# kaigu1997/gaussian_process_liouville_equation

Hardware: AMD Instinct MI355X
Metric: GP fit+predict ms/step (N samples, M grid pts) (lower is better)
Workload: dtype f64

## Files before the change

### gaussian_process_liouville_equation_amd/csrc/gple_capi.h

```cpp
#pragma once
#include <atomic>
#include <condition_variable>
#include <cstring>
#include <functional>
#include <limits>
#include <mutex>
#include <vector>

#include "gple_kernels.h"

using namespace gple;

struct gple_ctx: gple::Ctx
{
	struct PoolEntry
	{
		void* p;
		size_t bytes;
		bool used;
	};
	std::vector<PoolEntry> pool;
	std::mutex pool_mu;
	std::mutex call_mu;
	std::atomic<int> refs{1};
	std::atomic<bool> closed{false};

	double* acquire(size_t bytes, hipError_t* err)
	{
		std::lock_guard<std::mutex> lk(pool_mu);
		*err = hipSuccess;
		if (bytes == 0) bytes = 8;
		PoolEntry* best = nullptr;
		for (PoolEntry& e : pool)
			if (!e.used && e.bytes >= bytes && e.bytes <= 2 * bytes + 4096 && (!best || e.bytes < best->bytes)) best = &e;
		if (best)
		{
			best->used = true;
			return static_cast<double*>(best->p);
		}
		void* p = nullptr;
		*err = hipMalloc(&p, bytes);
		if (*err != hipSuccess) return nullptr;
		pool.push_back({p, bytes, true});
		return static_cast<double*>(p);
	}
	void give_back(void* p)
	{
		if (!p) return;
		std::lock_guard<std::mutex> lk(pool_mu);
		for (PoolEntry& e : pool)
			if (e.p == p) e.used = false;
	}
};

inline void ctx_retain(gple_ctx* c) { c->refs.fetch_add(1); }
inline void ctx_drop(gple_ctx* ctx)
{
	if (ctx->refs.fetch_sub(1) != 1) return;
	(void)hipSetDevice(ctx->device);
	(void)hipStreamSynchronize(ctx->stream);
	for (auto& e : ctx->pool) (void)hipFree(e.p);
	if (ctx->host_scalars) (void)hipHostFree(ctx->host_scalars);
	if (ctx->prune_stats) (void)hipFree(ctx->prune_stats);
	if (ctx->format_table) (void)hipFree(ctx->format_table);
	if (ctx->dag_flags) (void)hipFree(ctx->dag_flags);
	timer_collect(ctx);
	for (hipEvent_t e : ctx->ev_free) (void)hipEventDestroy(e);
	if (ctx->side_stream)
	{
		(void)hipStreamSynchronize(ctx->side_stream);
		(void)hipStreamDestroy(ctx->side_stream);
		for (hipEvent_t ev : ctx->side_forks) (void)hipEventDestroy(ev);
		if (ctx->side_join) (void)hipEventDestroy(ctx->side_join);
	}
	if (ctx->owns_stream) (void)hipStreamDestroy(ctx->stream);
	delete ctx;
}
#define GPLE_OPEN(ctx)                                  \
	do                                                  \
	{                                                   \
		if ((ctx)->closed.load()) return GPLE_ERR_STATE; \
	} while (0)
#define GPLE_CALL(ctx)                                             \
	std::lock_guard<std::mutex> gple_call_lk_((ctx)->call_mu); \
	GPLE_HIP((ctx), hipSetDevice((ctx)->device))

namespace gple
{
	constexpr int SDEV_N = 512;
	constexpr int HS_PRED_ERR = 512, HS_PRED_DERIV = 520, HS_NLML = 540;
	constexpr int SDEV_INFO = 31;
	constexpr int HS_FEW_XS = 600, HS_FEW_LAB = 640, HS_FEW_MEAN = 680, HS_FEW_VAR = 720, HS_FEW_CUT = 740;
	constexpr size_t FEW_HOST_POINTS = 16;

	struct Scratch
	{
		gple_ctx* ctx;
		double* p = nullptr;
		explicit Scratch(gple_ctx* c): ctx(c) {}
		Scratch(const Scratch&) = delete;
		~Scratch() { ctx->give_back(p); }
		hipError_t get(size_t doubles)
		{
			hipError_t e;
			p = ctx->acquire(doubles * sizeof(double), &e);
			return e;
		}
	};

	inline double nan_() { return std::numeric_limits<double>::quiet_NaN(); }

	inline hipError_t copy_in(hipStream_t s, double* dst, const double* src, size_t n, bool dev)
	{
		if (n == 0) return hipSuccess;
		return hipMemcpyAsync(dst, src, n * sizeof(double), dev ? hipMemcpyDeviceToDevice : hipMemcpyHostToDevice, s);
	}
	inline hipError_t copy_out(hipStream_t s, double* dst, const double* src, size_t n, bool dev)
	{
		if (n == 0 || dst == nullptr) return hipSuccess;
		return hipMemcpyAsync(dst, src, n * sizeof(double), dev ? hipMemcpyDeviceToDevice : hipMemcpyDeviceToHost, s);
	}

	struct Staged
	{
		Scratch buf;
		const bool dev;
		double* p = nullptr;
		double* host = nullptr;
		size_t n = 0;
		Staged(gple_ctx* c, bool device): buf(c), dev(device) {}
		hipError_t in(const double* src, size_t count)
		{
			p = const_cast<double*>(src);
			if (dev || !src) return hipSuccess;
			hipError_t e = buf.get(count);
			p = buf.p;
			return e == hipSuccess ? copy_in(buf.ctx->stream, p, src, count, false) : e;
		}
		hipError_t out(double* dst, size_t count)
		{
			p = dst;
			if (dev || !dst) return hipSuccess;
			host = dst, n = count;
			hipError_t e = buf.get(count);
			p = buf.p;
			return e;
		}
		hipError_t inout(double* a, size_t count)
		{
			if (!dev && a) host = a, n = count;
			return in(a, count);
		}
		hipError_t back() { return host ? copy_out(buf.ctx->stream, host, p, n, false) : hipSuccess; }
	};
}

struct FitCommon
{
	std::atomic<int> refs{1};
	gple_ctx* ctx = nullptr;
	int N = 0, Np = 0, n_total = 0;
	unsigned flags = 0;
	bool is_complex = false;
	double* Xt = nullptr;
	double* ys = nullptr;
	double* T = nullptr;
	double* v = nullptr;
	double* w = nullptr;
	double* wx = nullptr;
	double* W = nullptr;
	double* dv = nullptr;
	double sf = 1.0;
	double s0 = 1.0;
	DSpecSet dspec[6];
	double* sdev = nullptr;
	double s_host = 0.0;
	bool sc_ready = false;
	mutable std::atomic<bool> validated{false};
	mutable std::atomic<bool> recovered{false};
	mutable std::atomic<int> stale_uses{0};
	unsigned deriv_mask = 0xFFu;
	SEParamSet ps{};
	double self = 0.0;
	FitCommon() { std::memset(dspec, 0, sizeof(dspec)); }
	std::mutex lazy_mu;
	struct PointRequest
	{
		const double* x;
		double *mean, *var, *cut;
		int status;
		bool done;
	};
	mutable std::mutex point_mu;
	mutable std::condition_variable point_cv;
	mutable std::vector<PointRequest*> point_pending;
	mutable bool point_leader = false;

	~FitCommon()
	{
		if (!ctx) return;
		for (double* p : {Xt, ys, T, v, w, wx, W, dv, sdev}) ctx->give_back(p);
		ctx_drop(ctx);
	}
};
struct gple_real_fit: FitCommon
{
	double theta[4];
	gple_real_fit_scalars sc;
};
struct gple_complex_fit: FitCommon
{
	double theta[8];
	gple_complex_fit_scalars sc;
};

namespace gple
{
	constexpr unsigned PREDICT_NO_SYNC = 0x10000u;
	void predict_scalars_from_host(gple_ctx* ctx, bool has_labels, bool want_deriv, bool cplx, gple_predict_scalars* scalars);
	int predict_common(gple_ctx* ctx, const FitCommon* f, const double* Xs, size_t M, unsigned flags, const double* labels, double* prediction,
		double* variance, double* cutoff_prediction, gple_predict_scalars* scalars);
	inline bool own_outputs_written(int status, const FitCommon* f) { return status == GPLE_OK || (status == GPLE_ERR_TIMEOUT && f->validated.load()); }
	int real_fit_create_masked(gple_ctx* ctx, const double theta[4], const double* X, const double* y, int y_is_complex, size_t N, unsigned flags,
		unsigned deriv_mask, gple_real_fit_scalars* scalars, gple_real_fit** out);
	int complex_fit_create_masked(gple_ctx* ctx, const double theta[8], const double* X, const double* y, size_t N, unsigned flags, unsigned deriv_mask,
		gple_complex_fit_scalars* scalars, gple_complex_fit** out);
	int fit_predict(gple_ctx* ctx, const FitCommon* fit, const double* Xs, size_t M, unsigned flags, const double* labels, double* prediction,
		double* variance, double* cutoff_prediction, gple_predict_scalars* scalars);
	template <typename F>
	int fit_get_scalars(F* fit, decltype(F::sc)* out);
	template <typename F>
	int fit_release(F* fit);
	int note_give_up(gple_ctx* ctx, int attempt);
	int nlml_solve(gple_ctx* ctx, const double x[5], const double* X, const double* y, size_t N, Scratch& Xt, Scratch& yd, Scratch& T, Scratch& bvec,
		Scratch& info, int* n_out, bool dev = false);
	int nlml_gave_up(gple_ctx* ctx, int attempt, bool* again);
	using PointBatchEval = std::function<void(const std::vector<std::vector<double>>&, std::vector<double>&)>;
	int neldermead_speculative(const PointBatchEval& eval, unsigned n, const double* lb, const double* ub, const gple_opt_options* options, double* x,
		double* fmin, int* n_eval);
}
```

### gaussian_process_liouville_equation_amd/csrc/gple_capi.hip

```cpp
#include <algorithm>
#include <cmath>
#include <new>

#include "gple_capi.h"
#include "gple_debug.h"

namespace gple
{
	int record_hip_error(Ctx* ctx, hipError_t e, const char* what, const char* file, int line)
	{
		if (ctx)
		{
			std::lock_guard<std::mutex> lk(ctx->mu);
			ctx->last_error = std::string(hipGetErrorString(e)) + " in " + what + " (" + file + ":" + std::to_string(line) + ")";
		}
		(void)hipGetLastError();
		return e == hipErrorOutOfMemory ? GPLE_ERR_ALLOC : GPLE_ERR_HIP;
	}
	static bool take_event(Ctx* c, hipEvent_t* e)
	{
		if (!c->ev_free.empty())
		{
			*e = c->ev_free.back();
			c->ev_free.pop_back();
// ... 683 lines not shown
		}
		if (contracted_blocks) *contracted_blocks = h[0];
		if (seen_blocks) *seen_blocks = h[1];
		return GPLE_OK;
	}
	int gple_ctx_get_timing(gple_ctx* ctx, gple_timer which, double* last_ms, double* total_ms, long* count)
	{
		if (!ctx || static_cast<int>(which) < 0 || static_cast<int>(which) >= Ctx::NTIMERS) return GPLE_ERR_BAD_ARG;
		GPLE_OPEN(ctx);
		GPLE_CALL(ctx);
		GPLE_HIP(ctx, hipStreamSynchronize(ctx->stream));
		timer_collect(ctx);
		if (last_ms) *last_ms = ctx->t_last[which];
		if (total_ms) *total_ms = ctx->t_total[which];
		if (count) *count = ctx->t_count[which];
		return GPLE_OK;
	}

	int gple_real_gram(gple_ctx* ctx, const double theta[4], const double* left, size_t R, const double* right, size_t C,
		int same_features, unsigned flags, double* K, double* dK)
	{
		if (!ctx || !theta || !K || (R && !left) || (C && !right)) return GPLE_ERR_BAD_ARG;
		GPLE_OPEN(ctx);
		if (R == 0 || C == 0) return GPLE_OK;
		GPLE_CALL(ctx);
		const bool dev = flags & GPLE_IO_DEVICE;
		const SEParam p = make_se(theta[0] * theta[0], theta[3] * theta[3], theta[1], theta[2]);
		Staged l(ctx, dev), r(ctx, dev), k(ctx, dev), dk(ctx, dev);
		GPLE_HIP(ctx, l.in(left, 2 * R));
		GPLE_HIP(ctx, r.in(right, 2 * C));
		GPLE_HIP(ctx, k.out(K, R * C));
		GPLE_HIP(ctx, dk.out(dK, 4 * R * C));
		GPLE_HIP(ctx, launch_gram_rect(ctx->stream, l.p, (int)R, r.p, (int)C, same_features, p, theta[0], theta[3], k.p, dk.p));
		GPLE_HIP(ctx, k.back());
		GPLE_HIP(ctx, dk.back());
		if (!dev) GPLE_HIP(ctx, hipStreamSynchronize(ctx->stream));
		return GPLE_OK;
	}

	int gple_complex_gram(gple_ctx* ctx, const double theta[8], const double* left, size_t R, const double* right, size_t C, int same_features,
		unsigned flags, double* K, double* Kt, double* dK, double* dKt)
	{
		if (!ctx || !theta || !K || (R && !left) || (C && !right)) return GPLE_ERR_BAD_ARG;
		GPLE_OPEN(ctx);
		if (R == 0 || C == 0) return GPLE_OK;
		GPLE_CALL(ctx);
		const bool dev = flags & GPLE_IO_DEVICE;
		const size_t rc = R * C;
		Staged l(ctx, dev), r(ctx, dev), k(ctx, dev), kt(ctx, dev), dk(ctx, dev), dkt(ctx, dev);
		GPLE_HIP(ctx, l.in(left, 2 * R));
		GPLE_HIP(ctx, r.in(right, 2 * C));
		GPLE_HIP(ctx, k.out(K, rc));
		GPLE_HIP(ctx, kt.out(Kt, 2 * rc));
		GPLE_HIP(ctx, dk.out(dK, 8 * rc));
		GPLE_HIP(ctx, dkt.out(dKt, 16 * rc));
		GPLE_HIP(ctx, launch_complex_gram(ctx->stream, theta, l.p, (int)R, r.p, (int)C, same_features, k.p, kt.p, dk.p, dkt.p));
		for (Staged* o : {&k, &kt, &dk, &dkt}) GPLE_HIP(ctx, o->back());
		if (!dev) GPLE_HIP(ctx, hipStreamSynchronize(ctx->stream));
		return GPLE_OK;
	}

	int gple_cutoff_factor(gple_ctx* ctx, const double* prediction, int is_complex, const double* variance, size_t M, unsigned flags,
		double* factor)
	{
		if (!ctx || (M && (!prediction || !variance || !factor))) return GPLE_ERR_BAD_ARG;
		GPLE_OPEN(ctx);
		if (M == 0) return GPLE_OK;
		GPLE_CALL(ctx);
		const bool dev = flags & GPLE_IO_DEVICE;
		Staged p(ctx, dev), v(ctx, dev), f(ctx, dev);
		GPLE_HIP(ctx, p.in(prediction, is_complex ? 2 * M : M));
		GPLE_HIP(ctx, v.in(variance, M));
		GPLE_HIP(ctx, f.out(factor, M));
		GPLE_HIP(ctx, launch_cutoff(ctx->stream, p.p, is_complex, v.p, (int)M, f.p));
		GPLE_HIP(ctx, f.back());
		if (!dev) GPLE_HIP(ctx, hipStreamSynchronize(ctx->stream));
		return GPLE_OK;
	}

}

namespace
{
	static int fit_post(gple_ctx* ctx, gple_real_fit* f)
	{
		hipStream_t st = ctx->stream;
		const unsigned flags = f->flags;
		const double sf = f->theta[0], l0 = f->theta[1], l1 = f->theta[2], sn = f->theta[3];
		const size_t N = f->N;
		Scratch part(ctx);
		const size_t g = (N + 63) / 64;
		const bool avg = (flags & GPLE_CALC_AVERAGE) != 0;
		if (avg)
		{
			GPLE_HIP(ctx, part.get(g * g));
			GPLE_HIP(ctx, launch_quadform_partials(st, f->Xt, f->N, purity_aux(sf, l0, l1), f->v, f->v, -1, part.p));
		}
		GPLE_HIP(ctx, launch_real_fit_sums(st, f->Xt, f->ys, f->v, f->w, f->N, f->sdev + 1, avg ? part.p : nullptr, static_cast<int>(g * g), f->sdev + 6));
		if (flags & GPLE_CALC_DERIVATIVE) GPLE_TRY(real_fit_derivatives(ctx, f, sf, l0, l1, sn, flags));
		return GPLE_OK;
	}
	static int fit_post(gple_ctx* ctx, gple_complex_fit* f)
	{
		hipStream_t st = ctx->stream;
		const unsigned flags = f->flags;
		const double* theta = f->theta;
		const size_t N = f->N;
		const double sR = theta[1], lR0 = theta[2], lR1 = theta[3], sI = theta[4], lI0 = theta[5], lI1 = theta[6];
		hipLaunchKernelGGL(complex_fit_sums_kernel, dim3(1), dim3(1024), 0, st, f->ys, f->v, f->w, f->wx, f->N, f->Np, f->sdev + 1);
		GPLE_HIP(ctx, hipGetLastError());
		if (flags & GPLE_CALC_AVERAGE)
		{
			const ComplexAux a = complex_aux(theta);
			Scratch part(ctx);
			const size_t g = (N + 63) / 64;
			GPLE_HIP(ctx, part.get(g * g));
			const SEParam aR = purity_aux(sR, lR0, lR1), aI = purity_aux(sI, lI0, lI1), aC = purity_aux(a.sC, a.lC[0], a.lC[1]);
			const double *wr = f->v, *wi = f->v + f->Np;
			const SEParam ks[6] = {aR, aI, aC, aC, a.k[3], a.k[4]};
			const double* as[6] = {wr, wi, wr, wi, wr, wr};
			const double* bs[6] = {wr, wi, wr, wi, wi, wi};
			for (int q = 0; q < 6; ++q) GPLE_HIP(ctx, launch_quadform(st, f->Xt, f->N, ks[q], as[q], bs[q], -1, part.p, f->sdev + 8 + q));
		}
		if (flags & GPLE_CALC_DERIVATIVE) GPLE_TRY(complex_fit_derivatives(ctx, f, theta, flags));
		return GPLE_OK;
	}

	static int recover_fit(gple_ctx* ctx, FitCommon* f)
	{
		hipStream_t st = ctx->stream;
		f->recovered.store(true);
		for (double** p : {&f->W, &f->dv})
		{
			ctx->give_back(*p);
			*p = nullptr;
		}
		GPLE_HIP(ctx, hipMemsetAsync(f->sdev + SDEV_INFO, 0, sizeof(double), st));
		int status;
		{
			CholSchemeScope step(0);
			const int keep = ctx->chol_scheme;
			ctx->chol_scheme = -1;
			status = fit_factor(ctx, f);
			ctx->chol_scheme = keep;
		}
		if (status == GPLE_OK)
			status = f->is_complex ? fit_post(ctx, static_cast<gple_complex_fit*>(f)) : fit_post(ctx, static_cast<gple_real_fit*>(f));
		return status;
	}
	int validate_fit(gple_ctx* ctx, const FitCommon* fc)
	{
		FitCommon* f = const_cast<FitCommon*>(fc);
		hipStream_t st = ctx->stream;
		int info_i = 0;
		for (int attempt = 0;; ++attempt)
		{
			GPLE_HIP(ctx, hipMemcpyAsync(ctx->host_scalars, f->sdev, SDEV_N * 8, hipMemcpyDeviceToHost, st));
			GPLE_HIP(ctx, hipStreamSynchronize(st));
			std::memcpy(&info_i, ctx->host_scalars + SDEV_INFO, sizeof(int));
			if (info_i >= 0) break;
			GPLE_TRY(note_give_up(ctx, attempt));
			GPLE_TRY(recover_fit(ctx, f));
		}
		f->validated.store(true);
		return GPLE_OK;
	}
	int settle_fit(gple_ctx* ctx, const FitCommon* f)
	{
		if (!f->validated.load()) GPLE_TRY(validate_fit(ctx, f));
		if (!f->recovered.load()) return GPLE_OK;
		const int stale = f->stale_uses.exchange(0);
		if (stale == 0) return GPLE_OK;
		std::lock_guard<std::mutex> lk(ctx->mu);
		ctx->last_error = "the one-launch factorisation gave up waiting; the fit has been repeated with one launch per panel and is valid now, but "
			+ std::to_string(stale) + " call(s) enqueued on it before this synchronisation produced NaN: repeat them";
		return GPLE_ERR_TIMEOUT;
	}

	void closed_form_scalars(gple_real_fit* f, const double* h)
	{
		const unsigned flags = f->flags;
		const size_t N = f->N;
		const double sf = f->theta[0], l0 = f->theta[1], l1 = f->theta[2];
		const double s = h[0];
		gple_real_fit_scalars& sc = f->sc;
		{
			const double within = h[5] / static_cast<double>(N);
			sc.magnitude = within < 0 ? std::sqrt(-within) : std::sqrt(within);
		}
		if (flags & GPLE_CALC_ERROR) sc.error = h[1];
		if (flags & GPLE_CALC_AVERAGE)
		{
			const double GlobalFactor = 2.0 * M_PI;
			const double lprod = l0 * l1;
			sc.population = GlobalFactor * (sf * sf) * lprod * h[2] / s;
			sc.first_order_average[0] = GlobalFactor * (sf * sf) * lprod * h[3] / s;
			sc.first_order_average[1] = GlobalFactor * (sf * sf) * lprod * h[4] / s;
			const double PurityGlobal = (2.0 * M_PI) * M_PI;
			sc.purity = PurityGlobal * h[6] / (s * s);
		}
		if (flags & GPLE_CALC_DERIVATIVE)
		{
			if (flags & GPLE_CALC_ERROR)
				for (int ip = 0; ip < 4; ++ip) sc.error_derivative[ip] = h[16 + ip];
			if (flags & GPLE_CALC_AVERAGE)
			{
				const double ThisTimeFactor = (2.0 * M_PI) * (sf * sf) * (l0 * l1);
				const double ls[2] = {l0, l1};
				sc.population_derivative[0] = 0.0;
				for (int d = 0; d < 2; ++d) sc.population_derivative[1 + d] = ThisTimeFactor * (h[2] / ls[d] + h[21 + d]);
				sc.population_derivative[3] = ThisTimeFactor * h[23];
				for (double& d : sc.population_derivative) d /= s;
				const double PurityGlobal = (2.0 * M_PI) * M_PI;
				sc.purity_derivative[0] = 0.0;
				for (int d = 0; d < 2; ++d)
					sc.purity_derivative[1 + d] = ((h[6] / ls[d] + std::sqrt(2.0) * h[24 + d]) + 2.0 * h[26 + d]) * PurityGlobal;
				sc.purity_derivative[3] = 2.0 * PurityGlobal * h[28];
				for (double& d : sc.purity_derivative) d /= s * s;
			}
		}
	}
	void closed_form_scalars(gple_complex_fit* f, const double* h)
	{
		const unsigned flags = f->flags;
		const size_t N = f->N;
		const double* theta = f->theta;
		const double s0 = theta[0];
		double purity_sums[6];
		for (int q = 0; q < 6; ++q) purity_sums[q] = h[8 + q];
		const double s = h[0];
		gple_complex_fit_scalars& sc = f->sc;
		{
			const double within = h[2] / static_cast<double>(N);
			sc.magnitude = within < 0 ? std::sqrt(-within) : std::sqrt(within);
		}
		if (flags & GPLE_CALC_ERROR) sc.error = h[1];
		if (flags & GPLE_CALC_AVERAGE)
		{
			const double GlobalFactor = (2.0 * M_PI) * 2.0 * M_PI;
			const double ThisTimeFactor = GlobalFactor * ((s0 * s0) * (s0 * s0));
			const double qf = 0.25 * (2.0 * purity_sums[0] + 2.0 * purity_sums[1] + 2.0 * (purity_sums[2] + purity_sums[3])
				+ 4.0 * (purity_sums[4] + purity_sums[5]));
			sc.purity = ThisTimeFactor * qf / (s * s);
		}
		if (flags & GPLE_CALC_DERIVATIVE)
		{
			if (flags & GPLE_CALC_ERROR)
				for (int ip = 0; ip < 8; ++ip) sc.error_derivative[ip] = h[32 + ip];
			if (flags & GPLE_CALC_AVERAGE) complex_purity_derivative(theta, h, s, sc.purity_derivative);
		}
	}
	template <typename F>
	int fit_finalize(gple_ctx* ctx, F* f)
	{
		GPLE_TRY(validate_fit(ctx, f));
		timer_collect(ctx);
		const double* h = ctx->host_scalars;
		fill_nan_scalars(&f->sc);
		std::memcpy(&f->sc.info, h + SDEV_INFO, sizeof(int));
		f->s_host = f->sc.rescale_factor = h[0];
		closed_form_scalars(f, h);
		f->sc_ready = true;
		return settle_fit(ctx, f);
	}
	template <typename F>
	int fit_create(gple_ctx* ctx, F* f, const double* X, const double* y, int y_stride, size_t N, unsigned flags, decltype(F::sc)* scalars, F** out)
	{
		int status = fit_common(ctx, f, X, y, y_stride, N, flags);
		if (status == GPLE_OK)
		{
			status = fit_post(ctx, f);
			timer_stop(ctx, GPLE_TIMER_FIT);
		}
		if (status != GPLE_OK)
		{
			(void)hipStreamSynchronize(ctx->stream);
			delete f;
			return status;
		}
		if (scalars)
		{
			status = fit_finalize(ctx, f);
			if (status != GPLE_OK)
			{
				delete f;
				return status;
			}
			*scalars = f->sc;
		}
		*out = f;
		return GPLE_OK;
	}
	int fit_retain(FitCommon* fit)
	{
		if (!fit) return GPLE_ERR_BAD_ARG;
		fit->refs.fetch_add(1);
		return GPLE_OK;
	}
}

namespace gple
{
	int note_give_up(gple_ctx* ctx, int attempt)
	{
		ctx->dag_giveups += 1;
		if (attempt == 1)
		{
			std::lock_guard<std::mutex> lk(ctx->mu);
			ctx->last_error = "the factorisation gave up waiting (info = -1) and so did its repetition with one launch per panel";
			return GPLE_ERR_TIMEOUT;
		}
		ctx->dag_recoveries += 1;
		return GPLE_OK;
	}

	int real_fit_create_masked(gple_ctx* ctx, const double theta[4], const double* X, const double* y, int y_is_complex, size_t N,
		unsigned flags, unsigned deriv_mask, gple_real_fit_scalars* scalars, gple_real_fit** out)
	{
		if (!ctx || !theta || !X || !y || !out || N == 0 || N > (1u << 20)) return GPLE_ERR_BAD_ARG;
		GPLE_OPEN(ctx);
		*out = nullptr;
		GPLE_CALL(ctx);
		gple_real_fit* f = new (std::nothrow) gple_real_fit;
		if (!f) return GPLE_ERR_ALLOC;
		std::memcpy(f->theta, theta, sizeof(f->theta));
		const double sf = theta[0], sn = theta[3];
		f->ps.p[0] = f->ps.p[1] = f->ps.p[2] = make_se(sf * sf, sn * sn, theta[1], theta[2]);
		f->self = (sf * sf) * (1.0 + (sn * sn) * 1.0);
		f->sf = sf;
		f->deriv_mask = deriv_mask;
		return fit_create(ctx, f, X, y, y_is_complex ? 2 : 1, N, flags, scalars, out);
	}
	int complex_fit_create_masked(gple_ctx* ctx, const double theta[8], const double* X, const double* y, size_t N, unsigned flags,
		unsigned deriv_mask, gple_complex_fit_scalars* scalars, gple_complex_fit** out)
	{
		if (!ctx || !theta || !X || !y || !out || N == 0 || N > (1u << 19)) return GPLE_ERR_BAD_ARG;
		GPLE_OPEN(ctx);
		*out = nullptr;
		GPLE_CALL(ctx);
		gple_complex_fit* f = new (std::nothrow) gple_complex_fit;
		if (!f) return GPLE_ERR_ALLOC;
		f->is_complex = true;
		std::memcpy(f->theta, theta, sizeof(f->theta));
		const double s0 = theta[0], sR = theta[1], lR0 = theta[2], lR1 = theta[3], sI = theta[4], lI0 = theta[5], lI1 = theta[6],
					 sn = theta[7];
		const double ss0 = lR0 * lR0 + lI0 * lI0, ss1 = lR1 * lR1 + lI1 * lI1;
		const double sC = std::sqrt(sR * sI * ((2.0 * lR0 * lI0 / ss0) * (2.0 * lR1 * lI1 / ss1)));
		const double lC0 = std::sqrt(ss0 / 2.0), lC1 = std::sqrt(ss1 / 2.0);
		const double m2 = s0 * s0;
		f->ps.p[0] = make_se(m2 * (sR * sR), (sn * sn) / (2.0 * sR * sR), lR0, lR1);
		f->ps.p[1] = make_se(m2 * (sC * sC), 0.0, lC0, lC1);
		f->ps.p[2] = make_se(m2 * (sI * sI), (sn * sn) / (2.0 * sI * sI), lI0, lI1);
		f->self = m2 * (sR * sR * (1.0 + 0.0) + sI * sI * (1.0 + 0.0) + sn * sn * 1.0);
		f->s0 = s0;
		build_dspecs(theta, f->dspec);
		f->deriv_mask = deriv_mask;
		return fit_create(ctx, f, X, y, 2, N, flags, scalars, out);
	}
	template <typename F>
	int fit_get_scalars(F* fit, decltype(F::sc)* out)
	{
		if (!fit || !out) return GPLE_ERR_BAD_ARG;
		gple_ctx* ctx = fit->ctx;
		GPLE_CALL(ctx);
		const int status = fit->sc_ready ? settle_fit(ctx, fit) : fit_finalize(ctx, fit);
		if (fit->sc_ready) *out = fit->sc;
		return status;
	}
	template <typename F>
	int fit_release(F* fit)
	{
		if (!fit) return GPLE_OK;
		if (fit->refs.fetch_sub(1) == 1)
		{
			(void)hipSetDevice(fit->ctx->device);
			(void)hipStreamSynchronize(fit->ctx->stream);
			delete fit;
		}
		return GPLE_OK;
	}
	template int fit_get_scalars(gple_real_fit*, gple_real_fit_scalars*);
	template int fit_get_scalars(gple_complex_fit*, gple_complex_fit_scalars*);
	template int fit_release(gple_real_fit*);
	template int fit_release(gple_complex_fit*);

	void predict_scalars_from_host(gple_ctx* ctx, bool has_labels, bool want_deriv, bool cplx, gple_predict_scalars* scalars)
	{
		if (!scalars) return;
		if (has_labels) scalars->error = ctx->host_scalars[HS_PRED_ERR];
		if (want_deriv)
			for (int ip = 0; ip < (cplx ? 8 : 4); ++ip) scalars->error_derivative[ip] = ctx->host_scalars[HS_PRED_DERIV + ip];
	}
	static int predict_pass(gple_ctx* ctx, const FitCommon* f, const double* Xs, size_t M, unsigned flags, const double* labels,
		double* prediction, double* variance, double* cutoff_prediction, gple_predict_scalars* scalars);
	static bool predict_drains(unsigned flags, const double* labels) { return !(flags & PREDICT_NO_SYNC) && (!(flags & GPLE_IO_DEVICE) || labels); }
	int predict_common(gple_ctx* ctx, const FitCommon* f, const double* Xs, size_t M, unsigned flags, const double* labels,
		double* prediction, double* variance, double* cutoff_prediction, gple_predict_scalars* scalars)
	{
		if (scalars)
		{
			scalars->error = nan_();
			for (double& d : scalars->error_derivative) d = nan_();
		}
		if (M == 0) return GPLE_OK;
		if ((flags & GPLE_CALC_DERIVATIVE) && labels && !f->dv) return GPLE_ERR_STATE;
		GPLE_CALL(ctx);
		const bool unvalidated = !f->validated.load();
		GPLE_TRY(predict_pass(ctx, f, Xs, M, flags, labels, prediction, variance, cutoff_prediction, scalars));
		if (!predict_drains(flags, labels)) return GPLE_OK;
		if (unvalidated && f->recovered.load()) GPLE_TRY(predict_pass(ctx, f, Xs, M, flags, labels, prediction, variance, cutoff_prediction, scalars));
		return settle_fit(ctx, f);
	}
	static int predict_pass(gple_ctx* ctx, const FitCommon* f, const double* Xs, size_t M, unsigned flags, const double* labels,
		double* prediction, double* variance, double* cutoff_prediction, gple_predict_scalars* scalars)
	{
		const bool unvalidated = !f->validated.load();
		const bool want_deriv = (flags & GPLE_CALC_DERIVATIVE) && labels;
		hipStream_t st = ctx->stream;
		const bool dev = flags & GPLE_IO_DEVICE;
		const bool cplx = f->is_complex;
		const int Mi = static_cast<int>(M);
		const int Mh = static_cast<int>(round_up(M, 128));
		const int m_rows = cplx ? 2 * Mh : Mh;
		const size_t ow = cplx ? 2 : 1;
		Scratch q(ctx), mu(ctx), epart(ctx), dacc(ctx), dpart(ctx);
		Staged xs(ctx, dev), lab(ctx, dev), o_mean(ctx, dev), o_var(ctx, dev), o_cut(ctx, dev);
		timer_start(ctx, GPLE_TIMER_PREDICT);
		const double* xs_dev = Xs;
		const bool small_host = !dev && M <= FEW_HOST_POINTS && !(flags & PREDICT_NO_SYNC);
		if (small_host)
		{
			std::memcpy(ctx->host_scalars + HS_FEW_XS, Xs, 2 * M * sizeof(double));
			xs_dev = ctx->host_scalars + HS_FEW_XS;
		}
		else
		{
			GPLE_HIP(ctx, xs.in(Xs, 2 * M));
			xs_dev = xs.p;
		}
		GPLE_HIP(ctx, q.get(m_rows));
		GPLE_HIP(ctx, mu.get(m_rows));
		PredictArgs a{};
		a.Xs = xs_dev, a.M = Mi, a.m_rows = m_rows, a.m_split = cplx ? Mh : m_rows;
		a.Xt = f->Xt, a.N = f->N, a.n_total = f->n_total, a.n_split = cplx ? f->Np : f->n_total;
		a.T = f->T, a.ldt = f->n_total, a.v = f->v, a.q = q.p, a.mu = mu.p, a.ps = f->ps;
		if (!(flags & GPLE_PREDICT_FULL))
		{
			a.prune_thr = std::ldexp(f->self * f->ps.p[0].amp * f->ps.p[0].n2, cplx ? -57 : -56);
			if (!ctx->prune_stats)
			{
				GPLE_HIP(ctx, hipMalloc(reinterpret_cast<void**>(&ctx->prune_stats), 4 * sizeof(unsigned long long)));
				GPLE_HIP(ctx, hipMemsetAsync(ctx->prune_stats, 0, 4 * sizeof(unsigned long long), st));
			}
			a.prune_stats = ctx->prune_stats;
		}
		if (want_deriv)
		{
			GPLE_HIP(ctx, dacc.get((cplx ? 15 : 7) * static_cast<size_t>(m_rows)));
			a.dv = f->dv, a.dacc = dacc.p;
// ... 412 lines not shown
```

### gaussian_process_liouville_equation_amd/csrc/gple_chol.hip

```cpp
#include <algorithm>
#include <cstdio>
#include <cstdlib>
#include <functional>
#include <map>
#include <mutex>
#include <string>
#include <utility>
#include <vector>

#include "gple_internal.h"

namespace gple
{
	namespace
	{
		constexpr int NB = CHOL_NB;

		__device__ __forceinline__ double rsqrt_newton(double d)
		{
			const double r = __builtin_amdgcn_rsq(d);
			const double e = fma(-(d * r), r, 1.0);
			return fma(r, e * fma(0.375, e, 0.5), r);
		}

// ... 1643 lines not shown
	{
		const InvWork w = chol_inverse_work_split(n);
		return w.prod + w.side + w.main + 64 + static_cast<size_t>(NB) * n + w.tt;
	}
	static double* chol_work_tt(double* work, int n)
	{
		const InvWork w = chol_inverse_work_split(n);
		return w.tt ? work + w.prod + w.side + w.main + 64 + static_cast<size_t>(NB) * n : nullptr;
	}
	static double* chol_work_pa(double* work, int n)
	{
		const InvWork w = chol_inverse_work_split(n);
		return work + w.prod + w.side + w.main + 64;
	}
	static int tri_tile(long m, long ncols, long batch, int origin)
	{
		const int t = gemm_pick_tile(m, ncols, batch, true);
		return t == 128 && origin % 128 ? 64 : t;
	}
	namespace
	{
		__global__ void spin_kernel(long long ticks)
		{
			const long long t0 = wall_clock64();
			while (wall_clock64() - t0 < ticks) __builtin_amdgcn_s_sleep(8);
		}
	}
	static hipError_t pick_side_stream(Ctx* ctx, hipStream_t main_stream)
	{
		static const int side_prio = [] {
			int lo = 0, hi = 0;
			return hipDeviceGetStreamPriorityRange(&lo, &hi) == hipSuccess ? lo : 0;
		}();
		constexpr int MAX_CANDIDATES = 8;
		constexpr long long SPIN_TICKS = 10000;
		hipError_t e;
		hipEvent_t ev[3] = {nullptr, nullptr, nullptr};
		for (hipEvent_t& x : ev)
			if ((e = hipEventCreate(&x)) != hipSuccess) return e;
		std::vector<hipStream_t> rejected;
		hipStream_t chosen = nullptr;
		for (int attempt = 0; attempt < MAX_CANDIDATES && !chosen; ++attempt)
		{
			hipStream_t cand = nullptr;
			if ((e = hipStreamCreateWithPriority(&cand, hipStreamNonBlocking, side_prio)) != hipSuccess) break;
			ctx->side_attempts = attempt + 1;
			float t_main = 0.f, t_side = 0.f, t_ref = 0.f;
			bool ok = hipEventRecord(ev[0], main_stream) == hipSuccess && hipStreamWaitEvent(cand, ev[0], 0) == hipSuccess;
			if (ok)
			{
				hipLaunchKernelGGL(spin_kernel, dim3(1), dim3(64), 0, main_stream, SPIN_TICKS);
				hipLaunchKernelGGL(spin_kernel, dim3(1), dim3(64), 0, cand, SPIN_TICKS);
				ok = hipEventRecord(ev[1], main_stream) == hipSuccess && hipEventRecord(ev[2], cand) == hipSuccess && hipStreamSynchronize(cand) == hipSuccess
					&& hipStreamSynchronize(main_stream) == hipSuccess && hipEventElapsedTime(&t_main, ev[0], ev[1]) == hipSuccess
					&& hipEventElapsedTime(&t_side, ev[0], ev[2]) == hipSuccess;
			}
			if (ok)
			{
				ok = hipEventRecord(ev[0], main_stream) == hipSuccess;
				hipLaunchKernelGGL(spin_kernel, dim3(1), dim3(64), 0, main_stream, SPIN_TICKS);
				ok = ok && hipEventRecord(ev[1], main_stream) == hipSuccess && hipStreamSynchronize(main_stream) == hipSuccess
					&& hipEventElapsedTime(&t_ref, ev[0], ev[1]) == hipSuccess;
			}
			if (!ok || std::max(t_main, t_side) < 1.6f * t_ref)
			{
				chosen = cand;
				ctx->side_overlaps = ok;
			}
			else rejected.push_back(cand);
		}
		if (!chosen && !rejected.empty())
		{
			chosen = rejected.back();
			rejected.pop_back();
		}
		for (hipStream_t r : rejected) (void)hipStreamDestroy(r);
		for (hipEvent_t x : ev) (void)hipEventDestroy(x);
		(void)hipGetLastError();
		if (!chosen) return hipErrorOutOfMemory;
		ctx->side_stream = chosen;
		return hipSuccess;
	}

	hipError_t chol_inverse_factor(Ctx* ctx, hipStream_t s, double* A, long lda, int n, double* T, long ldt, int* info, double* work, double* uvec)
	{
		if (n % NB) return hipErrorInvalidValue;
		const std::vector<int>& marks = chol_marks(n);
		if (marks.empty())
		{
			if (chol_dag_inverse_inside(n)) return potrf_lower(s, A, lda, n, T, ldt, info, uvec, ctx, work, chol_work_pa(work, n));
			hipError_t e = potrf_lower(s, A, lda, n, T, ldt, info, uvec, ctx, nullptr, chol_work_pa(work, n));
			if (e != hipSuccess) return e;
			return trtri_lower_from_diag(s, A, lda, T, ldt, n, work);
		}
		hipError_t e;
		if (!ctx->side_stream)
		{
			if ((e = pick_side_stream(ctx, s)) != hipSuccess) return e;
			if ((e = hipEventCreateWithFlags(&ctx->side_join, hipEventDisableTiming)) != hipSuccess) return e;
		}
		while (ctx->side_forks.size() < marks.size())
		{
			hipEvent_t ev;
			if ((e = hipEventCreateWithFlags(&ev, hipEventDisableTiming)) != hipSuccess) return e;
			ctx->side_forks.push_back(ev);
		}
		hipStream_t side = ctx->side_stream;
		const InvWork iw = chol_inverse_work_split(n);
		const int f1 = marks.front();
		const long ldw = n - f1;
		double* w_all = work;
		double* w_side = work + iw.prod;
		double* w_main = work + iw.prod + iw.side;
		auto tree = [&](hipStream_t st, int g0, int g1, double* w_tree) -> hipError_t {
			return trtri_lower_from_diag(st, A + g0 + static_cast<long>(g0) * lda, lda, T + g0 + static_cast<long>(g0) * ldt, ldt, g1 - g0, w_tree, g0);
		};
		auto w_accumulate = [&](hipStream_t st, int g0, int g1) -> hipError_t {
			GemmDesc g{};
			g.A = A + g1 + static_cast<long>(g0) * lda, g.lda = lda, g.ldb = ldt, g.ldc = ldw;
			g.M = n - g1, g.K = g1 - g0, g.batch = 1, g.alpha = 1.0;
			g.lower_only = 0, g.a_kmajor = false, g.b_kmajor = true, g.c_trans = false;
			if (g0 > 0)
			{
				g.B = T + g0, g.C = w_all + (g1 - f1), g.N = g0, g.beta = 1.0, g.krange = K_FULL;
				const hipError_t er = launch_gemm(st, g, gemm_pick_tile(g.M, g.N, 1, false));
				if (er != hipSuccess) return er;
			}
			g.B = T + g0 + static_cast<long>(g0) * ldt, g.C = w_all + (g1 - f1) + static_cast<long>(g0) * ldw, g.N = g1 - g0, g.beta = 0.0, g.krange = K_GE_N;
			return launch_gemm(st, g, tri_tile(g.M, g.N, 1, g0));
		};
		auto t_product = [&](hipStream_t st, int g0, int g1) -> hipError_t {
			GemmDesc g{};
			g.A = T + g0 + static_cast<long>(g0) * ldt, g.lda = ldt, g.B = w_all + (g0 - f1), g.ldb = ldw, g.C = T + g0, g.ldc = ldt;
			g.M = g1 - g0, g.N = g0, g.K = g1 - g0, g.batch = 1, g.alpha = -1.0, g.beta = 0.0;
			g.krange = K_LE_M, g.lower_only = 0, g.a_kmajor = false, g.b_kmajor = true, g.c_trans = false;
			return launch_gemm(st, g, tri_tile(g1 - g0, g0, 1, g0));
		};
		int done = 0;
		size_t nfork = 0;
		const bool use_dag = chol_dag_scheme();
		const std::vector<int> dag_cuts = use_dag ? chol_dag_cuts(n, &marks) : std::vector<int>{};
		const std::function<hipError_t(int)> on_final = [&](int j) -> hipError_t {
			hipError_t er;
			hipEvent_t ev = ctx->side_forks[nfork++];
			if ((er = hipEventRecord(ev, s)) != hipSuccess) return er;
			if ((er = hipStreamWaitEvent(side, ev, 0)) != hipSuccess) return er;
			if (!(use_dag && chol_block_inverse_inside(n, done, j, dag_cuts)) && (er = tree(side, done, j, w_side)) != hipSuccess) return er;
			if (done > 0 && (er = t_product(side, done, j)) != hipSuccess) return er;
			if ((er = w_accumulate(side, done, j)) != hipSuccess) return er;
			done = j;
			return hipSuccess;
		};
		DagState dst{};
		dst.pa = chol_work_pa(work, n);
		dst.tt = chol_work_tt(work, n);
		if (use_dag && (e = dag_state(ctx, s, n, dst)) != hipSuccess) return e;
		if ((e = potrf_columns(s, A, lda, n, T, ldt, info, 0, n, uvec, &marks, &on_final, use_dag ? &dst : nullptr)) != hipSuccess) return e;
		if ((e = hipEventRecord(ctx->side_join, side)) != hipSuccess) return e;
		if (!(use_dag && chol_block_inverse_inside(n, done, n, dag_cuts)) && (e = tree(s, done, n, w_main)) != hipSuccess) return e;
		if ((e = hipStreamWaitEvent(s, ctx->side_join, 0)) != hipSuccess) return e;
		return t_product(s, done, n);
	}

	void chol_layout(int n, std::vector<int>& bounds, std::vector<int>& forks, size_t& work_doubles)
	{
		bounds = chol_block_bounds(n);
		forks = chol_marks(n);
		work_doubles = chol_inverse_work_doubles(n);
	}

	hipError_t lauum_full(hipStream_t s, const double* T, long ldt, double* W, long ldw, int n)
	{
		GemmDesc g{};
		g.A = T, g.lda = ldt, g.B = T, g.ldb = ldt, g.C = W, g.ldc = ldw;
		g.M = n, g.N = n, g.K = n, g.batch = 1, g.alpha = 1.0, g.beta = 0.0;
		g.krange = K_GE_MAX_MN, g.lower_only = 1, g.a_kmajor = true, g.b_kmajor = true, g.c_trans = false;
		hipError_t e = launch_gemm(s, g, gemm_pick_tile(n, n, 1, true));
		if (e != hipSuccess) return e;
		hipLaunchKernelGGL(mirror_lower_kernel, dim3(n / 32, n / 32), dim3(256), 0, s, W, ldw, n);
		return hipGetLastError();
	}
}
```

### gaussian_process_liouville_equation_amd/csrc/gple_internal.h

```cpp
#pragma once
#include <hip/hip_runtime.h>

#include <cstddef>
#include <cstdint>
#include <mutex>
#include <string>
#include <vector>

#include "../../include/gple.h"

namespace gple
{
	constexpr int NPAD = 256;
	constexpr int CHOL_NB = 64;

	inline size_t round_up(size_t n, size_t m) { return (n + m - 1) / m * m; }

	struct Ctx;
	int record_hip_error(Ctx* ctx, hipError_t e, const char* what, const char* file, int line);
#define GPLE_HIP(ctx, expr)                                                        \
	do                                                                             \
	{                                                                              \
		hipError_t gple_e_ = (expr);                                               \
		if (gple_e_ != hipSuccess) return gple::record_hip_error((ctx), gple_e_, #expr, __FILE_NAME__, __LINE__); \
	} while (0)
#define GPLE_TRY(expr)                        \
	do                                        \
	{                                         \
		int gple_s_ = (expr);                 \
		if (gple_s_ != GPLE_OK) return gple_s_; \
	} while (0)

	struct DevBuf
	{
		void* p = nullptr;
		size_t bytes = 0;
		DevBuf() = default;
		DevBuf(const DevBuf&) = delete;
		DevBuf& operator=(const DevBuf&) = delete;
		~DevBuf() { release(); }
		hipError_t alloc(size_t nbytes)
		{
			release();
			if (nbytes == 0) return hipSuccess;
			hipError_t e = hipMalloc(&p, nbytes);
			if (e == hipSuccess) bytes = nbytes;
			else p = nullptr;
			return e;
		}
		hipError_t ensure(size_t nbytes) { return nbytes <= bytes ? hipSuccess : alloc(nbytes); }
		void release()
		{
			if (p) (void)hipFree(p);
			p = nullptr;
			bytes = 0;
		}
		double* d() const { return static_cast<double*>(p); }
	};

	struct Ctx
	{
		int device = 0;
		hipStream_t stream = nullptr;
		bool owns_stream = false;
		std::string last_error;
		std::mutex mu;
		hipStream_t side_stream = nullptr;
		int side_attempts = 0;
		bool side_overlaps = false;
		hipEvent_t side_join = nullptr;
		int* dag_flags = nullptr;
		size_t dag_flags_ints = 0;
		int dag_epoch = 0;
		int chol_scheme = -1, dag_poll_limit = 0, dag_blocks = 0;
		const char* last_contraction = "";
		int fused_small = -1;
		int rownorm_pipe = -1;
		long dag_giveups = 0, dag_recoveries = 0;
		std::vector<hipEvent_t> side_forks;
		double* host_scalars = nullptr;
		unsigned long long* prune_stats = nullptr;
		unsigned long long* format_table = nullptr;
		bool format_slots = false;
		struct TimedSpan
		{
			int which;
			hipEvent_t e0, e1;
		};
		bool timing = false;
		std::vector<hipEvent_t> ev_free;
		std::vector<TimedSpan> pending;
		static constexpr int NTIMERS = 10;
		TimedSpan open_span[NTIMERS] = {};
		double t_last[NTIMERS] = {}, t_total[NTIMERS] = {};
		long t_count[NTIMERS] = {};
	};
	void chunk_timer_start(Ctx* c);
	void chunk_timer_stop(Ctx* c);
	void timer_start(Ctx* c, int which);
	void timer_stop(Ctx* c, int which);
	void timer_collect(Ctx* c);

	enum KRange
	{
		K_FULL = 0,
		K_GE_N = 1,
		K_LE_M = 2,
		K_GE_MAX_MN = 3
	};
	struct GemmDesc
	{
		const double* A;
		long lda;
		long strideA;
		const double* B;
		long ldb;
		long strideB;
		double* C;
		long ldc;
		long strideC;
		int M, N, K;
		int batch;
		double alpha, beta;
		int krange;
		int lower_only;
		bool a_kmajor, b_kmajor, c_trans;
	};
	hipError_t launch_gemm(hipStream_t s, const GemmDesc& d, int tile);
	int gemm_pick_tile(long m, long n, long batch, bool triangular);

	struct CholSchemeScope
	{
		explicit CholSchemeScope(int scheme);
		~CholSchemeScope();
		CholSchemeScope(const CholSchemeScope&) = delete;
		int saved;
	};
	hipError_t potrf_lower(hipStream_t s, double* A, long lda, int n, double* T, long ldt, int* info, double* uvec = nullptr, Ctx* ctx = nullptr,
		double* tt = nullptr, double* pa = nullptr);
	void chol_layout(int n, std::vector<int>& bounds, std::vector<int>& forks, size_t& work_doubles);
	hipError_t debug_potrf_step(hipStream_t s, double* A, long lda, double* T, long ldt, int* info, long long* stamps, int pend, int below);
	hipError_t trtri_lower_from_diag(hipStream_t s, const double* L, long ldl, double* T, long ldt, int n, double* work, int origin = 0);
	size_t chol_inverse_work_doubles(int n);
	hipError_t chol_inverse_factor(Ctx* ctx, hipStream_t s, double* A, long lda, int n, double* T, long ldt, int* info, double* work,
		double* uvec = nullptr);
	hipError_t lauum_full(hipStream_t s, const double* T, long ldt, double* W, long ldw, int n);
}
```

Baseline: 64.20.

## Run fit post-processing sums on side stream and rebalance Cholesky gemm streams

Moves the fit's post-processing kernels (quadform partials and fit sums) onto the side stream, forked by an event and joined before the host reads the scalars, so they can overlap with derivative work on the main stream. The quadform partial buffer is now held per fit rather than taken from scratch each call. In the Cholesky inverse, the w_accumulate gemm goes to the main stream when the DAG kernel already handles the block inverse. The change also adds a timeline probe script and extra event lifetime handling, which bring new cross-stream ordering risks.

```diff
diff --git a/gaussian_process_liouville_equation_amd/csrc/gple_capi.h b/gaussian_process_liouville_equation_amd/csrc/gple_capi.h
--- a/gaussian_process_liouville_equation_amd/csrc/gple_capi.h
+++ b/gaussian_process_liouville_equation_amd/csrc/gple_capi.h
@@ -70,9 +70,10 @@
 	{
 		(void)hipStreamSynchronize(ctx->side_stream);
 		(void)hipStreamDestroy(ctx->side_stream);
-		for (hipEvent_t ev : ctx->side_forks) (void)hipEventDestroy(ev);
-		if (ctx->side_join) (void)hipEventDestroy(ctx->side_join);
-	}
+	}
+	for (hipEvent_t ev : ctx->side_forks) (void)hipEventDestroy(ev);
+	for (hipEvent_t ev : {ctx->side_join, ctx->post_fork, ctx->post_done})
+		if (ev) (void)hipEventDestroy(ev);
 	if (ctx->owns_stream) (void)hipStreamDestroy(ctx->stream);
 	delete ctx;
 }
@@ -174,6 +175,8 @@
 	double s0 = 1.0;
 	DSpecSet dspec[6];
 	double* sdev = nullptr;
+	double* qpart = nullptr;
+	bool post_aside = false;
 	double s_host = 0.0;
 	bool sc_ready = false;
 	mutable std::atomic<bool> validated{false};
@@ -199,7 +202,7 @@
 	~FitCommon()
 	{
 		if (!ctx) return;
-		for (double* p : {Xt, ys, T, v, w, wx, W, dv, sdev}) ctx->give_back(p);
+		for (double* p : {Xt, ys, T, v, w, wx, W, dv, sdev, qpart}) ctx->give_back(p);
 		ctx_drop(ctx);
 	}
 };
diff --git a/gaussian_process_liouville_equation_amd/csrc/gple_capi.hip b/gaussian_process_liouville_equation_amd/csrc/gple_capi.hip
--- a/gaussian_process_liouville_equation_amd/csrc/gple_capi.hip
+++ b/gaussian_process_liouville_equation_amd/csrc/gple_capi.hip
@@ -789,46 +789,75 @@
 
 namespace
 {
+	static int post_stream(gple_ctx* ctx, FitCommon* f, hipStream_t* st)
+	{
+		GPLE_HIP(ctx, ensure_side_stream(ctx, ctx->stream));
+		GPLE_HIP(ctx, hipEventRecord(ctx->post_fork, ctx->stream));
+		GPLE_HIP(ctx, hipStreamWaitEvent(ctx->side_stream, ctx->post_fork, 0));
+		*st = ctx->side_stream;
+		f->post_aside = true;
+		return GPLE_OK;
+	}
+	static int post_stream_done(gple_ctx* ctx, FitCommon* f)
+	{
+		if (f->post_aside) GPLE_HIP(ctx, hipEventRecord(ctx->post_done, ctx->side_stream));
+		return GPLE_OK;
+	}
+	static int fit_post_join(gple_ctx* ctx, const FitCommon* f)
+	{
+		if (f->post_aside) GPLE_HIP(ctx, hipStreamWaitEvent(ctx->stream, ctx->post_done, 0));
+		return GPLE_OK;
+	}
 	static int fit_post(gple_ctx* ctx, gple_real_fit* f)
 	{
-		hipStream_t st = ctx->stream;
+		hipStream_t st;
 		const unsigned flags = f->flags;
 		const double sf = f->theta[0], l0 = f->theta[1], l1 = f->theta[2], sn = f->theta[3];
 		const size_t N = f->N;
-		Scratch part(ctx);
 		const size_t g = (N + 63) / 64;
 		const bool avg = (flags & GPLE_CALC_AVERAGE) != 0;
+		if (avg && !f->qpart)
+		{
+			hipError_t e;
+			f->qpart = ctx->acquire(g * g * sizeof(double), &e);
+			GPLE_HIP(ctx, e);
+		}
+		GPLE_TRY(post_stream(ctx, f, &st));
 		if (avg)
-		{
-			GPLE_HIP(ctx, part.get(g * g));
-			GPLE_HIP(ctx, launch_quadform_partials(st, f->Xt, f->N, purity_aux(sf, l0, l1), f->v, f->v, -1, part.p));
-		}
-		GPLE_HIP(ctx, launch_real_fit_sums(st, f->Xt, f->ys, f->v, f->w, f->N, f->sdev + 1, avg ? part.p : nullptr, static_cast<int>(g * g), f->sdev + 6));
+			GPLE_HIP(ctx, launch_quadform_partials(st, f->Xt, f->N, purity_aux(sf, l0, l1), f->v, f->v, -1, f->qpart));
+		GPLE_HIP(ctx, launch_real_fit_sums(st, f->Xt, f->ys, f->v, f->w, f->N, f->sdev + 1, avg ? f->qpart : nullptr, static_cast<int>(g * g), f->sdev + 6));
+		GPLE_TRY(post_stream_done(ctx, f));
 		if (flags & GPLE_CALC_DERIVATIVE) GPLE_TRY(real_fit_derivatives(ctx, f, sf, l0, l1, sn, flags));
 		return GPLE_OK;
 	}
 	static int fit_post(gple_ctx* ctx, gple_complex_fit* f)
 	{
-		hipStream_t st = ctx->stream;
+		hipStream_t st;
 		const unsigned flags = f->flags;
 		const double* theta = f->theta;
 		const size_t N = f->N;
 		const double sR = theta[1], lR0 = theta[2], lR1 = theta[3], sI = theta[4], lI0 = theta[5], lI1 = theta[6];
+		const size_t g = (N + 63) / 64;
+		if ((flags & GPLE_CALC_AVERAGE) && !f->qpart)
+		{
+			hipError_t e;
+			f->qpart = ctx->acquire(g * g * sizeof(double), &e);
+			GPLE_HIP(ctx, e);
+		}
+		GPLE_TRY(post_stream(ctx, f, &st));
 		hipLaunchKernelGGL(complex_fit_sums_kernel, dim3(1), dim3(1024), 0, st, f->ys, f->v, f->w, f->wx, f->N, f->Np, f->sdev + 1);
 		GPLE_HIP(ctx, hipGetLastError());
 		if (flags & GPLE_CALC_AVERAGE)
 		{
 			const ComplexAux a = complex_aux(theta);
-			Scratch part(ctx);
-			const size_t g = (N + 63) / 64;
-			GPLE_HIP(ctx, part.get(g * g));
 			const SEParam aR = purity_aux(sR, lR0, lR1), aI = purity_aux(sI, lI0, lI1), aC = purity_aux(a.sC, a.lC[0], a.lC[1]);
 			const double *wr = f->v, *wi = f->v + f->Np;
 			const SEParam ks[6] = {aR, aI, aC, aC, a.k[3], a.k[4]};
 			const double* as[6] = {wr, wi, wr, wi, wr, wr};
 			const double* bs[6] = {wr, wi, wr, wi, wi, wi};
-			for (int q = 0; q < 6; ++q) GPLE_HIP(ctx, launch_quadform(st, f->Xt, f->N, ks[q], as[q], bs[q], -1, part.p, f->sdev + 8 + q));
-		}
+			for (int q = 0; q < 6; ++q) GPLE_HIP(ctx, launch_quadform(st, f->Xt, f->N, ks[q], as[q], bs[q], -1, f->qpart, f->sdev + 8 + q));
+		}
+		GPLE_TRY(post_stream_done(ctx, f));
 		if (flags & GPLE_CALC_DERIVATIVE) GPLE_TRY(complex_fit_derivatives(ctx, f, theta, flags));
 		return GPLE_OK;
 	}
@@ -862,6 +891,7 @@
 		int info_i = 0;
 		for (int attempt = 0;; ++attempt)
 		{
+			GPLE_TRY(fit_post_join(ctx, f));
 			GPLE_HIP(ctx, hipMemcpyAsync(ctx->host_scalars, f->sdev, SDEV_N * 8, hipMemcpyDeviceToHost, st));
 			GPLE_HIP(ctx, hipStreamSynchronize(st));
 			std::memcpy(&info_i, ctx->host_scalars + SDEV_INFO, sizeof(int));
@@ -982,6 +1012,7 @@
 		if (status != GPLE_OK)
 		{
 			(void)hipStreamSynchronize(ctx->stream);
+			if (f->post_aside) (void)hipStreamSynchronize(ctx->side_stream);
 			delete f;
 			return status;
 		}
@@ -1082,6 +1113,7 @@
 		{
 			(void)hipSetDevice(fit->ctx->device);
 			(void)hipStreamSynchronize(fit->ctx->stream);
+			if (fit->post_aside) (void)hipStreamSynchronize(fit->ctx->side_stream);
 			delete fit;
 		}
 		return GPLE_OK;
diff --git a/gaussian_process_liouville_equation_amd/csrc/gple_chol.hip b/gaussian_process_liouville_equation_amd/csrc/gple_chol.hip
--- a/gaussian_process_liouville_equation_amd/csrc/gple_chol.hip
+++ b/gaussian_process_liouville_equation_amd/csrc/gple_chol.hip
@@ -1749,6 +1749,15 @@
 		return hipSuccess;
 	}
 
+	hipError_t ensure_side_stream(Ctx* ctx, hipStream_t main_stream)
+	{
+		if (ctx->side_stream) return hipSuccess;
+		hipError_t e;
+		for (hipEvent_t* ev : {&ctx->side_join, &ctx->post_fork, &ctx->post_done})
+			if (*ev == nullptr && (e = hipEventCreateWithFlags(ev, hipEventDisableTiming)) != hipSuccess) return e;
+		return pick_side_stream(ctx, main_stream);
+	}
+
 	hipError_t chol_inverse_factor(Ctx* ctx, hipStream_t s, double* A, long lda, int n, double* T, long ldt, int* info, double* work, double* uvec)
 	{
 		if (n % NB) return hipErrorInvalidValue;
@@ -1761,11 +1770,7 @@
 			return trtri_lower_from_diag(s, A, lda, T, ldt, n, work);
 		}
 		hipError_t e;
-		if (!ctx->side_stream)
-		{
-			if ((e = pick_side_stream(ctx, s)) != hipSuccess) return e;
-			if ((e = hipEventCreateWithFlags(&ctx->side_join, hipEventDisableTiming)) != hipSuccess) return e;
-		}
+		if ((e = ensure_side_stream(ctx, s)) != hipSuccess) return e;
 		while (ctx->side_forks.size() < marks.size())
 		{
 			hipEvent_t ev;
@@ -1782,7 +1787,7 @@
 		auto tree = [&](hipStream_t st, int g0, int g1, double* w_tree) -> hipError_t {
 			return trtri_lower_from_diag(st, A + g0 + static_cast<long>(g0) * lda, lda, T + g0 + static_cast<long>(g0) * ldt, ldt, g1 - g0, w_tree, g0);
 		};
-		auto w_accumulate = [&](hipStream_t st, int g0, int g1) -> hipError_t {
+		auto w_accumulate = [&](hipStream_t st, hipStream_t st_own, int g0, int g1) -> hipError_t {
 			GemmDesc g{};
 			g.A = A + g1 + static_cast<long>(g0) * lda, g.lda = lda, g.ldb = ldt, g.ldc = ldw;
 			g.M = n - g1, g.K = g1 - g0, g.batch = 1, g.alpha = 1.0;
@@ -1794,7 +1799,7 @@
 				if (er != hipSuccess) return er;
 			}
 			g.B = T + g0 + static_cast<long>(g0) * ldt, g.C = w_all + (g1 - f1) + static_cast<long>(g0) * ldw, g.N = g1 - g0, g.beta = 0.0, g.krange = K_GE_N;
-			return launch_gemm(st, g, tri_tile(g.M, g.N, 1, g0));
+			return launch_gemm(st_own, g, tri_tile(g.M, g.N, 1, g0));
 		};
 		auto t_product = [&](hipStream_t st, int g0, int g1) -> hipError_t {
 			GemmDesc g{};
@@ -1812,9 +1817,11 @@
 			hipEvent_t ev = ctx->side_forks[nfork++];
 			if ((er = hipEventRecord(ev, s)) != hipSuccess) return er;
 			if ((er = hipStreamWaitEvent(side, ev, 0)) != hipSuccess) return er;
-			if (!(use_dag && chol_block_inverse_inside(n, done, j, dag_cuts)) && (er = tree(side, done, j, w_side)) != hipSuccess) return er;
+			const bool inside = use_dag && chol_block_inverse_inside(n, done, j, dag_cuts);
+			if (!inside && (er = tree(side, done, j, w_side)) != hipSuccess) return er;
 			if (done > 0 && (er = t_product(side, done, j)) != hipSuccess) return er;
-			if ((er = w_accumulate(side, done, j)) != hipSuccess) return er;
+			const bool own_on_main = inside && done > 0;
+			if ((er = w_accumulate(side, own_on_main ? s : side, done, j)) != hipSuccess) return er;
 			done = j;
 			return hipSuccess;
 		};
diff --git a/gaussian_process_liouville_equation_amd/csrc/gple_internal.h b/gaussian_process_liouville_equation_amd/csrc/gple_internal.h
--- a/gaussian_process_liouville_equation_amd/csrc/gple_internal.h
+++ b/gaussian_process_liouville_equation_amd/csrc/gple_internal.h
@@ -78,6 +78,7 @@
 		int rownorm_pipe = -1;
 		long dag_giveups = 0, dag_recoveries = 0;
 		std::vector<hipEvent_t> side_forks;
+		hipEvent_t post_fork = nullptr, post_done = nullptr;
 		double* host_scalars = nullptr;
 		unsigned long long* prune_stats = nullptr;
 		unsigned long long* format_table = nullptr;
@@ -144,5 +145,6 @@
 	size_t chol_inverse_work_doubles(int n);
 	hipError_t chol_inverse_factor(Ctx* ctx, hipStream_t s, double* A, long lda, int n, double* T, long ldt, int* info, double* work,
 		double* uvec = nullptr);
+	hipError_t ensure_side_stream(Ctx* ctx, hipStream_t main_stream);
 	hipError_t lauum_full(hipStream_t s, const double* T, long ldt, double* W, long ldw, int n);
 }
diff --git a/probes/fit_timeline.py b/probes/fit_timeline.py
--- /dev/null
+++ b/probes/fit_timeline.py
@@ -0,0 +1,42 @@
+import csv, re, sys
+
+rows = list(csv.DictReader(open(sys.argv[1])))
+rows.sort(key=lambda r: int(r["Start_Timestamp"]))
+first = max(i for i, r in enumerate(rows) if "prep_labels" in r["Kernel_Name"])
+sel = rows[first:]
+t0 = int(sel[0]["Start_Timestamp"])
+main = sel[0]["Stream_Id"]
+
+
+def short(name):
+    return re.sub(r"\(anonymous namespace\)::|gple::|void ", "", name).split("(")[0]
+
+
+us = lambda t: (int(t) - t0) / 1e3
+print(f"# {sys.argv[2] if len(sys.argv) > 2 else 'fit timeline'}\n")
+print("Last of the traced fits; times in µs from the start of the fit's first kernel; stream M = the context's stream, S = its side stream.\n")
+print("| stream | kernel | workgroups | LDS B | start | end | µs |")
+print("|---|---|---|---|---|---|---|")
+for r in sel:
+    wg = (int(r["Grid_Size_X"]) // int(r["Workgroup_Size_X"])) * (int(r["Grid_Size_Y"]) // int(r["Workgroup_Size_Y"])) * (int(r["Grid_Size_Z"]) // int(r["Workgroup_Size_Z"]))
+    print(f"| {'M' if r['Stream_Id'] == main else 'S'} | `{short(r['Kernel_Name'])}` | {wg} | {r['LDS_Block_Size']} | {us(r['Start_Timestamp']):.1f} | {us(r['End_Timestamp']):.1f} | "
+          f"{(int(r['End_Timestamp']) - int(r['Start_Timestamp'])) / 1e3:.1f} |")
+mrows = [r for r in sel if r["Stream_Id"] == main]
+end = max(us(r["End_Timestamp"]) for r in sel)
+main_end = max(us(r["End_Timestamp"]) for r in mrows)
+print(f"\nFit: {end:.1f} µs to the end of its last kernel ({main_end:.1f} µs on the main stream).\n")
+print("## Main stream without a `potrf_dag_kernel`\n")
+print("| from | to | µs | what the main stream runs meanwhile |")
+print("|---|---|---|---|")
+spine = [(us(r["Start_Timestamp"]), us(r["End_Timestamp"])) for r in mrows if "potrf_dag_kernel" in r["Kernel_Name"]]
+edges = [0.0] + [x for se in spine for x in se] + [main_end]
+total = 0.0
+for a, b in zip(edges[0::2], edges[1::2]):
+    if b - a <= 0:
+        continue
+    inside = [f"`{short(r['Kernel_Name'])}` {(int(r['End_Timestamp']) - int(r['Start_Timestamp'])) / 1e3:.1f}" for r in mrows
+              if "potrf_dag_kernel" not in r["Kernel_Name"] and a - 1.0 <= us(r["Start_Timestamp"]) < b - 1.0]
+    busy = min(b - a, sum(float(x.rsplit(" ", 1)[1]) for x in inside))
+    print(f"| {a:.1f} | {b:.1f} | {b - a:.1f} | {', '.join(inside) or '—'}; idle {b - a - busy:.1f} |")
+    total += b - a
+print(f"\n`potrf_dag_kernel` launches: {', '.join(f'{b - a:.1f}' for a, b in spine)} µs = {sum(b - a for a, b in spine):.1f} µs; the main stream outside them: {total:.1f} µs.")
```

Result: no change. 64.39 (+0.3%).
